# davidtweedle/gptq-svd

Hardware: AMD Instinct MI355X
Metric: weight-cols quantized/sec at d_in=4096 (higher is better)
Workload: dtype f64+f32; 1 GPU; single synthetic 4096x4096 Hessian per rank, full solver (eigh, rank rule, pivot order, U, 4-bit asym g128 quantize, pack); n=4096, m=4096, calib_rows=3072, rank_k=3058, threshold_method=energy, block_size=1024, parallelism=independent layer per rank x1

## Files before the change

### gptq-svd_amd/csrc/band.h

```cpp
#pragma once
#include <algorithm>
#include <type_traits>
#include <vector>

#include "common.h"

namespace tg {

constexpr int SB_B = 32;
constexpr int SB_C = 256;
constexpr int SB_LV = 6;
constexpr int PQR_NWMAX = 256;
constexpr int PQR_BC_DOUBLES = 8192;

struct SbLevel {
  int rows, nc;
  size_t yoff, toff;
};
struct SbPanel {
  int p, r0, m, nl;
  SbLevel L[SB_LV];
};

struct SbPlan {
  std::vector<SbPanel> panels;
  size_t ytotal = 0, ttotal = 0;
  int ncmax = 1;
  bool single = false;
  explicit SbPlan(int n);
};

struct SbBufs {
  double *Y, *T;
  double *YT, *X, *G, *M;
  double *YTl[SB_LV];
  double *R[2];
  double *Gr, *U;
  double *Xs;
  double *Zg, *P, *Mz;
  double *Bst;
  double *V2;
  double *T2;
  unsigned *prog;
  double *pq_part, *pq_bc;
  unsigned *pq_ctl;
  unsigned *xm_tick;
  double *xm_xpart;
};

int pqr_rows_per_thread(int m);
hipError_t panel_qr(hipStream_t st, double *A, int lda, int p, int r0, int m, double *Y,
                    double *YT, double *T, double *part, double *bc, unsigned *cnt,
                    unsigned *tmo);

int sb_smax(int n);
size_t sb2st_prog_words(int n);
size_t sb2st_t2_count(int n);

inline size_t pq_ctl_words(int n) { return 4 + 4 * size_t(std::max(1, n / SB_B + 1)); }
inline size_t xm_mflag_off(int n) { return size_t(n) / 256 + 7; }
inline size_t xm_cbt_off(int n) { return size_t(n) / 256 + 8; }
inline size_t xm_tick_words(int n) { return xm_cbt_off(n) + size_t(n) / 16 + 2; }
inline size_t xm_xpart_doubles(int n) { return 8 * (size_t(n) + 32) * 32; }

template <class A>
void sb_layout(A &ar, int n, int kmax, const SbPlan &pl, SbBufs *bp) {
  SbBufs d{};
  SbBufs &b = bp ? *bp : d;
  const size_t w = size_t(pl.ncmax) * SB_B;
  auto take = [&](double *&dst, size_t cnt) {
    if constexpr (std::is_same_v<A, Arena>) dst = ar.template take<double>(cnt);
    else ar.template take<double>(cnt);
  };
  take(b.Y, pl.ytotal + 1);
  take(b.T, pl.ttotal + 1);
  take(b.YT, size_t(n) * SB_B);
  for (int l = 1; l < SB_LV; ++l) take(b.YTl[l], w * SB_B);
  take(b.X, size_t(n) * w);
  take(b.G, w * w);
  take(b.M, w * w);
  take(b.R[0], w * SB_B);
  take(b.R[1], w * SB_B);
  take(b.Gr, w * n);
  take(b.U, std::max({w * n, (size_t(n) / 16 + size_t(n) / 256 + 2) * 1024,
                      (size_t(n) / 32 + size_t(n) / 1024 + 2) * 5 * 1024}));
  take(b.Xs, w * w);
  take(b.Zg, w * kmax);
  take(b.P, w * kmax);
  take(b.Mz, w * kmax);
  const size_t nsw = size_t(std::max(1, n - 2)), smax = size_t(sb_smax(n));
  take(b.Bst, size_t(n) * 2 * SB_B);
  take(b.V2, nsw * smax * SB_B);
  take(b.T2, sb2st_t2_count(n));
  if constexpr (std::is_same_v<A, Arena>) b.prog = ar.template take<unsigned>(sb2st_prog_words(n));
  else ar.template take<unsigned>(sb2st_prog_words(n));
  const size_t npart = std::max<size_t>(std::max<size_t>(2 * PQR_NWMAX + 2, size_t(n) / SB_C + 2),
                                        size_t(n) / 128 + 2) * 1024;
  take(b.pq_part, npart);
  take(b.pq_bc, PQR_BC_DOUBLES);
  if constexpr (std::is_same_v<A, Arena>) b.pq_ctl = ar.template take<unsigned>(pq_ctl_words(n));
  else ar.template take<unsigned>(pq_ctl_words(n));
  if constexpr (std::is_same_v<A, Arena>) b.xm_tick = ar.template take<unsigned>(xm_tick_words(n));
  else ar.template take<unsigned>(xm_tick_words(n));
  take(b.xm_xpart, xm_xpart_doubles(n));
}

hipError_t sy2sb(hipStream_t st, double *A, int lda, int n, const SbPlan &pl, const SbBufs &b);
hipError_t sy2sb_timed_out(hipStream_t st, const SbPlan &pl, const SbBufs &b, bool *tmo);
hipError_t sb2st(hipStream_t st, const double *A, int lda, int n, double *Bst, double *V2,
                 unsigned *prog, double *d, double *e);
hipError_t sb2st_stalled(hipStream_t st, int n, const unsigned *prog, bool *stalled,
                         bool *broken = nullptr);
hipError_t sb_apply_q2(hipStream_t st, int n, double *Z, int k, const double *V2,
                       double *T2);
hipError_t sb_q2_tfactors(hipStream_t st, int n, const double *V2, double *T2);
hipError_t side_fork(hipStream_t st, hipStream_t *side);
hipError_t side_join(hipStream_t st);
bool sb_apply_few_ok(const SbPlan &pl, int n, int k);
size_t sb_apply_few_scratch(const SbPlan &pl, int n, int k);
hipError_t sb_apply_few(hipStream_t st, int n, double *Z, int k, const SbPlan &pl,
                        const SbBufs &b, void *dev, bool *timed_out);
hipError_t sb_apply_q1(hipStream_t st, int n, double *Z, int k, const SbPlan &pl,
                       const SbBufs &b);

}
```

### gptq-svd_amd/csrc/band.hip

```cpp
#include <algorithm>
#include <cmath>
#include <cstdio>
#include <cstdlib>
#include <utility>
#include <vector>

#include "band.h"
#include "gemm64.h"
#include "reduce.h"
#include "spin.h"

namespace tg {

SbPlan::SbPlan(int n) {
  ncmax = std::max(1, n / SB_C);
  const char *e = getenv("TG_SB_TSQR");
  single = !(e && e[0] == '1') && pqr_rows_per_thread(n) > 0;
  int p = 0;
  while (p + SB_B < n - 1) {
    SbPanel P{};
    P.p = p;
    P.r0 = p + SB_B;
    P.m = n - P.r0;
    if (single) {
// ... 972 lines not shown
      if constexpr (NBC == 1)
        if (g.fuse_w) xm_fused_w<NBC>(g, r0, xs, ys, &red[XW - 4][0][0]);
      return;
    }
    for (int e = tid; e < ne; e += 64 * XW) Cs[e] = xm_sum(g.gpart, 0, NG, e, NP * 1024);
  }
  __syncthreads();
  for (int e = tid; e < SB_B * SB_B; e += 64 * XW) {
    const int a = e >> 5, c = e & 31;
    double v = 0.0;
    for (int k = 0; k <= a; ++k) v = fma(Ts[k * SB_B + a], Cs[k * SB_B + c], v);
    if (NBC == 1 && g.fuse_w)
      __hip_atomic_store(&g.M[e], v, __ATOMIC_RELAXED, __HIP_MEMORY_SCOPE_AGENT);
    else
      g.M[e] = v;
  }
  if (NBC == 1 && g.fuse_w) {
    asm volatile("s_waitcnt vmcnt(0)" ::: "memory");
    __syncthreads();
    if (tid == 0) {
      tg::ctl_reset(&g.tick[grp]);
      if (NG > 1) tg::ctl_reset(&g.tick[NG]);
      __hip_atomic_store(g.mflag, g.epoch, __ATOMIC_RELAXED, __HIP_MEMORY_SCOPE_AGENT);
    }
    if constexpr (NBC == 1) xm_fused_w<NBC>(g, r0, xs, ys, &red[XW - 4][0][0]);
    return;
  }
  if (pp) {
    const double *Ps = Cs + 1024, *Qs = Cs + 2048, *E1 = Cs + 3072, *E2 = Cs + 4096;
    for (int e = tid; e < 2048; e += 64 * XW) g.PQ[e] = Cs[1024 + e];
    __syncthreads();
    for (int e = tid; e < SB_B * SB_B; e += 64 * XW) {
      const int a = e >> 5, c = e & 31;
      double v = 0.0;
#pragma unroll 8
      for (int k = 0; k < SB_B; ++k) v = fma(E1[a * SB_B + k], Ps[k * SB_B + c], v);
#pragma unroll 8
      for (int k = 0; k < SB_B; ++k) v = fma(E2[a * SB_B + k], Qs[k * SB_B + c], v);
      Cs[e] = v;
    }
    __syncthreads();
    for (int e = tid; e < SB_B * SB_B; e += 64 * XW) {
      const int a = e >> 5, c = e & 31;
      double v = 0.0;
      for (int k = 0; k <= a; ++k) v = fma(Ts[k * SB_B + a], Cs[k * SB_B + c], v);
      g.PQ[2048 + e] = v;
    }
  }
  if (tid == 0) {
    tg::ctl_reset(&g.tick[grp]);
    if (NG > 1) tg::ctl_reset(&g.tick[NG]);
  }
}

constexpr int WU_R = 16;
__global__ __launch_bounds__(256) void w_update_kernel(const double *__restrict__ Y,
                                                       double *__restrict__ X, int m,
                                                       const double *__restrict__ M) {
  __shared__ double2 Ms[SB_B][SB_B / 2];
  const int tid = threadIdx.x;
  const int r = blockIdx.x * WU_R + (tid >> 4), c2 = tid & 15;
  const int rc = min(r, m - 1);
  double2 y[SB_B / 2];
#pragma unroll
  for (int h = 0; h < SB_B / 2; ++h) y[h] = reinterpret_cast<const double2 *>(Y + int64_t(rc) * SB_B)[h];
  const double2 x = reinterpret_cast<const double2 *>(X + int64_t(rc) * SB_B)[c2];
  for (int e = tid; e < SB_B * SB_B / 2; e += 256)
    Ms[e >> 4][e & 15] = reinterpret_cast<const double2 *>(M)[e];
  __syncthreads();
  double v0 = 0.0, v1 = 0.0;
#pragma unroll
  for (int h = 0; h < SB_B / 2; ++h) {
    const double2 a = Ms[2 * h][c2], b = Ms[2 * h + 1][c2];
    v0 = fma(y[h].x, a.x, v0);
    v1 = fma(y[h].x, a.y, v1);
    v0 = fma(y[h].y, b.x, v0);
    v1 = fma(y[h].y, b.y, v1);
  }
  if (r < m)
    reinterpret_cast<double2 *>(X + int64_t(r) * SB_B)[c2] =
        make_double2(fma(-0.5, v0, x.x), fma(-0.5, v1, x.y));
}

constexpr int WT = 64, WK = 2 * SB_B, WP = 4;
struct YW2 {
  const double *Y[2], *W[2];
};
template <int NP>
__global__ __launch_bounds__(256, 2) void syr2k_w_kernel(double *__restrict__ A, int64_t lda, int m,
                                                         YW2 yw) {
  __shared__ double Aop[WK][WT + WP];
  __shared__ double Bop[WK][WT + WP];
  const int b = blockIdx.x;
  int I = int((sqrt(8.0 * b + 1.0) - 1.0) * 0.5);
  while ((I + 1) * (I + 2) / 2 <= b) ++I;
  while (I * (I + 1) / 2 > b) --I;
  const int J = b - I * (I + 1) / 2;
  const int tm = I * WT, tn = J * WT;
  const int tid = threadIdx.x, lane = tid & 63, wid = tid >> 6;
  const int wm = wid >> 1, wn = wid & 1;
  double old[2][2][4];
#pragma unroll
  for (int i = 0; i < 2; ++i)
#pragma unroll
    for (int j = 0; j < 2; ++j)
#pragma unroll
      for (int r = 0; r < 4; ++r) {
        const int gi = min(tm + wm * 32 + i * 16 + (lane >> 4) + 4 * r, m - 1);
        const int gj = min(tn + wn * 32 + j * 16 + (lane & 15), m - 1);
        old[i][j][r] = A[int64_t(gi) * lda + gj];
      }
  doublex4 acc[2][2];
#pragma unroll
  for (int i = 0; i < 2; ++i)
#pragma unroll
    for (int j = 0; j < 2; ++j) acc[i][j] = doublex4{0.0, 0.0, 0.0, 0.0};
#pragma unroll
  for (int pp = 0; pp < NP; ++pp) {
    if (pp > 0) __syncthreads();
    const double *Y = yw.Y[pp], *W = yw.W[pp];
    {
      const int rl = tid >> 2, k0 = (tid & 3) * 8;
      const int gr = min(tm + rl, m - 1), gc = min(tn + rl, m - 1);
      const bool okr = tm + rl < m, okc = tn + rl < m;
      double2 v[4][4];
      const double *src[4] = {Y + int64_t(gr) * SB_B + k0, W + int64_t(gr) * SB_B + k0,
                              W + int64_t(gc) * SB_B + k0, Y + int64_t(gc) * SB_B + k0};
#pragma unroll
      for (int o = 0; o < 4; ++o)
#pragma unroll
        for (int h = 0; h < 4; ++h) v[o][h] = reinterpret_cast<const double2 *>(src[o])[h];
#pragma unroll
      for (int h = 0; h < 4; ++h) {
        const int k = k0 + 2 * h;
        Aop[k][rl] = okr ? v[0][h].x : 0.0;
        Aop[k + 1][rl] = okr ? v[0][h].y : 0.0;
        Aop[SB_B + k][rl] = okr ? v[1][h].x : 0.0;
        Aop[SB_B + k + 1][rl] = okr ? v[1][h].y : 0.0;
        Bop[k][rl] = okc ? v[2][h].x : 0.0;
        Bop[k + 1][rl] = okc ? v[2][h].y : 0.0;
        Bop[SB_B + k][rl] = okc ? v[3][h].x : 0.0;
        Bop[SB_B + k + 1][rl] = okc ? v[3][h].y : 0.0;
      }
    }
    __syncthreads();
#pragma unroll
    for (int kq = 0; kq < WK; kq += 4) {
      double af[2], bf[2];
#pragma unroll
      for (int i = 0; i < 2; ++i) af[i] = Aop[kq + (lane >> 4)][wm * 32 + i * 16 + (lane & 15)];
#pragma unroll
      for (int j = 0; j < 2; ++j) bf[j] = Bop[kq + (lane >> 4)][wn * 32 + j * 16 + (lane & 15)];
#pragma unroll
      for (int i = 0; i < 2; ++i)
#pragma unroll
        for (int j = 0; j < 2; ++j)
          acc[i][j] = __builtin_amdgcn_mfma_f64_16x16x4f64(af[i], bf[j], acc[i][j], 0, 0, 0);
    }
  }
  __syncthreads();
  double(*Tt)[WT + 1] = reinterpret_cast<double(*)[WT + 1]>(&Aop[0][0]);
  static_assert(WK * (WT + WP) >= WT * (WT + 1), "mirror tile must fit");
#pragma unroll
  for (int i = 0; i < 2; ++i)
#pragma unroll
    for (int j = 0; j < 2; ++j)
#pragma unroll
      for (int r = 0; r < 4; ++r) {
        const int li = wm * 32 + i * 16 + (lane >> 4) + 4 * r, lj = wn * 32 + j * 16 + (lane & 15);
        const int gi = tm + li, gj = tn + lj;
        if (gi < m && gj < m && gi >= gj) {
          const double v = old[i][j][r] - acc[i][j][r];
          A[int64_t(gi) * lda + gj] = v;
          if (tm != tn) Tt[li][lj] = v;
          else if (gi != gj) A[int64_t(gj) * lda + gi] = v;
        }
      }
  if (tm != tn) {
    __syncthreads();
    for (int idx = tid; idx < WT * WT; idx += 256) {
      const int lc = idx >> 6, lr = idx & 63;
      if (tn + lc < m && tm + lr < m) A[int64_t(tn + lc) * lda + tm + lr] = Tt[lr][lc];
    }
  }
}

__device__ __forceinline__ void syr2k_tile(int b, int &tm, int &tn) {
  int I = int((sqrt(8.0 * b + 1.0) - 1.0) * 0.5);
  while ((I + 1) * (I + 2) / 2 <= b) ++I;
  while (I * (I + 1) / 2 > b) --I;
  tm = I * WT;
  tn = (b - I * (I + 1) / 2) * WT;
}
template <int NP>
__global__ __launch_bounds__(256, 2) void syr2k_wp_kernel(double *__restrict__ A, int64_t lda,
                                                          int m, YW2 yw, int ntiles) {
  __shared__ double Aop[WK][WT + WP];
  __shared__ double Bop[WK][WT + WP];
  const int tid = threadIdx.x, lane = tid & 63, wid = tid >> 6;
  const int wm = wid >> 1, wn = wid & 1;
  int b = blockIdx.x;
  if (b >= ntiles) return;
  auto load_old = [&](int tb, double (&o)[2][2][4]) __attribute__((always_inline)) {
    int tm, tn;
    syr2k_tile(tb, tm, tn);
#pragma unroll
    for (int i = 0; i < 2; ++i)
#pragma unroll
      for (int j = 0; j < 2; ++j)
#pragma unroll
        for (int r = 0; r < 4; ++r) {
          const int gi = min(tm + wm * 32 + i * 16 + (lane >> 4) + 4 * r, m - 1);
          const int gj = min(tn + wn * 32 + j * 16 + (lane & 15), m - 1);
          o[i][j][r] = A[int64_t(gi) * lda + gj];
        }
  };
  double old[2][2][4], nold[2][2][4];
  load_old(b, old);
  for (; b < ntiles; b += gridDim.x) {
    int tm, tn;
    syr2k_tile(b, tm, tn);
    const int rl = tid >> 2, k0 = (tid & 3) * 8;
    const int gr = min(tm + rl, m - 1), gc = min(tn + rl, m - 1);
    const bool okr = tm + rl < m, okc = tn + rl < m;
    doublex4 acc[2][2];
#pragma unroll
    for (int i = 0; i < 2; ++i)
#pragma unroll
      for (int j = 0; j < 2; ++j) acc[i][j] = doublex4{0.0, 0.0, 0.0, 0.0};
#pragma unroll
    for (int pp = 0; pp < NP; ++pp) {
      __syncthreads();
      const double *Y = yw.Y[pp], *W = yw.W[pp];
      double2 v[4][4];
      {
        const double *src[4] = {Y + int64_t(gr) * SB_B + k0, W + int64_t(gr) * SB_B + k0,
                                W + int64_t(gc) * SB_B + k0, Y + int64_t(gc) * SB_B + k0};
#pragma unroll
        for (int o = 0; o < 4; ++o)
#pragma unroll
          for (int h = 0; h < 4; ++h) v[o][h] = reinterpret_cast<const double2 *>(src[o])[h];
      }
      if (pp == 0) {
        __builtin_amdgcn_sched_barrier(0);
        const int bn = b + int(gridDim.x);
        if (bn < ntiles) load_old(bn, nold);
        __builtin_amdgcn_sched_barrier(0);
      }
#pragma unroll
      for (int h = 0; h < 4; ++h) {
        const int k = k0 + 2 * h;
        Aop[k][rl] = okr ? v[0][h].x : 0.0;
        Aop[k + 1][rl] = okr ? v[0][h].y : 0.0;
        Aop[SB_B + k][rl] = okr ? v[1][h].x : 0.0;
        Aop[SB_B + k + 1][rl] = okr ? v[1][h].y : 0.0;
        Bop[k][rl] = okc ? v[2][h].x : 0.0;
        Bop[k + 1][rl] = okc ? v[2][h].y : 0.0;
        Bop[SB_B + k][rl] = okc ? v[3][h].x : 0.0;
        Bop[SB_B + k + 1][rl] = okc ? v[3][h].y : 0.0;
      }
      __syncthreads();
#pragma unroll
      for (int kq = 0; kq < WK; kq += 4) {
        double af[2], bf[2];
#pragma unroll
        for (int i = 0; i < 2; ++i) af[i] = Aop[kq + (lane >> 4)][wm * 32 + i * 16 + (lane & 15)];
#pragma unroll
        for (int j = 0; j < 2; ++j) bf[j] = Bop[kq + (lane >> 4)][wn * 32 + j * 16 + (lane & 15)];
#pragma unroll
        for (int i = 0; i < 2; ++i)
#pragma unroll
          for (int j = 0; j < 2; ++j)
            acc[i][j] = __builtin_amdgcn_mfma_f64_16x16x4f64(af[i], bf[j], acc[i][j], 0, 0, 0);
      }
    }
    __syncthreads();
// ... 266 lines not shown
  if (e != hipSuccess) return e;
  SideStream &x = ss[dev & 63];
  if (!x.s) {
    if ((e = hipStreamCreateWithFlags(&x.s, hipStreamNonBlocking)) != hipSuccess) return e;
    for (int i = 0; i < 2; ++i) {
      if ((e = hipEventCreateWithFlags(&x.ev0[i], hipEventDisableTiming)) != hipSuccess) return e;
      if ((e = hipEventCreateWithFlags(&x.ev1[i], hipEventDisableTiming)) != hipSuccess) return e;
    }
    if ((e = hipEventCreateWithFlags(&x.evj, hipEventDisableTiming)) != hipSuccess) return e;
  }
  out = &x;
  return hipSuccess;
}

hipError_t side_fork(hipStream_t st, hipStream_t *side) {
  SideStream *ss = nullptr;
  TG_CHK(side_stream(ss));
  TG_CHK(hipEventRecord(ss->evj, st));
  TG_CHK(hipStreamWaitEvent(ss->s, ss->evj, 0));
  *side = ss->s;
  return hipSuccess;
}
hipError_t side_join(hipStream_t st) {
  SideStream *ss = nullptr;
  TG_CHK(side_stream(ss));
  TG_CHK(hipEventRecord(ss->evj, ss->s));
  TG_CHK(hipStreamWaitEvent(st, ss->evj, 0));
  return hipSuccess;
}

static int xm_nbc(int m) {
  const char *fx = getenv("TG_XM_NBC");
  return fx ? (atoi(fx) == 2 ? 2 : 1) : (m >= XM_WIDE ? 2 : 1);
}
template <int NBC>
static int xm_resident() {
  static int cached[64] = {0};
  int dev = 0;
  if (hipGetDevice(&dev) != hipSuccess || dev < 0 || dev >= 64) return 0;
  if (cached[dev] == 0) {
    int ncu = 0, occ = 0;
    if (hipDeviceGetAttribute(&ncu, hipDeviceAttributeMultiprocessorCount, dev) != hipSuccess)
      ncu = 0;
    if (hipOccupancyMaxActiveBlocksPerMultiprocessor(&occ, xm_kernel<NBC>, 64 * XW, 0) !=
        hipSuccess)
      occ = 0;
    cached[dev] = std::max(0, ncu) * std::max(0, occ);
    if (cached[dev] == 0) cached[dev] = -1;
  }
  return std::max(0, cached[dev]);
}
static int xm_ksplit(int m, int G, int nbc) {
  const char *e = getenv("TG_XM_KSPLIT");
  int S = (e && atoi(e) > 0) ? atoi(e) : (nbc == 1 || G >= 1536 ? 1 : cdiv(1536, G));
  S = std::max(1, std::min(8, S));
  while (S > 1 && cdiv(m, S) < 4 * 32) --S;
  return S;
}
static hipError_t launch_xm(hipStream_t st, double *A22, int lda, int m, const double *YT,
                            const double *Yp, const double *Tp, double *X, const SbBufs &b,
                            int n, const double *Ya = nullptr, const double *Wa = nullptr,
                            double *PQ = nullptr, unsigned epoch = 0, bool *fused = nullptr) {
  const int nbc = xm_nbc(m);
  if (Ya && nbc != 2) return hipErrorInvalidValue;
  const int G = cdiv(m, XR * nbc), np = Ya ? 5 : 1;
  const int S = xm_ksplit(m, G, nbc), kc = cdiv(cdiv(m, S), 32) * 32;
  unsigned *mflag = b.xm_tick + xm_mflag_off(n);
  const char *xs = getenv("TG_XM_ASM");
  const int asm_loads = !(xs && xs[0] == '0');
  const char *fw = getenv("TG_XM_FUSE_W");
  const bool fuse = epoch > 0 && !Ya && nbc == 1 && (fw && fw[0] == '1') &&
                    2 * G * S <= xm_resident<1>();
  if (fused) *fused = fuse;
  static const unsigned long long tmo_ticks = spin_timeout_ticks("TG_XM_TIMEOUT_TICKS");
  XmArgs xa{A22, int64_t(lda), m, YT, Yp, Tp, X, b.U, b.U + size_t(G) * np * 1024, b.M,
            b.xm_tick, asm_loads, Ya, Wa, PQ, fuse ? 1 : 0,
            mflag, epoch, b.pq_ctl, tmo_ticks, S, kc, b.xm_xpart, b.xm_tick + xm_cbt_off(n)};
  if (nbc == 2) hipLaunchKernelGGL(xm_kernel<2>, dim3(G * S), dim3(64 * XW), 0, st, xa);
  else hipLaunchKernelGGL(xm_kernel<1>, dim3(G * S), dim3(64 * XW), 0, st, xa);
  return hipGetLastError();
}

constexpr int PAIR_MIN_ALL = 256, PAIR_MIN = 6144;

static hipError_t sy2sb_single(hipStream_t st, double *A, int lda, int n, const SbPlan &pl,
                               const SbBufs &b) {
  TG_CHK(hipMemsetAsync(b.pq_ctl, 0, sizeof(unsigned) * pq_ctl_words(n), st));
  TG_CHK(hipMemsetAsync(b.xm_tick, 0, sizeof(unsigned) * xm_tick_words(n), st));
  const int np = int(pl.panels.size());
  const char *pe = getenv("TG_SB_PAIR");
  const bool pairs = !(pe && pe[0] == '0') && pl.ncmax >= 2;
  const int pair_min = (pe && pe[0] == '1') ? PAIR_MIN_ALL : PAIR_MIN;
  const char *ps = getenv("TG_SYR2K_PERSIST");
  const bool persist = !(ps && ps[0] == '0');
  const XcdInfo xi = xcd_info();
  const int ncu = std::max(1, xi.xcds * xi.cus_per_xcd);
  SideStream *ss = nullptr;
  const char *psd = getenv("TG_SB_PAIR_SIDE");
  const bool pair_side = psd && psd[0] == '1';
  double *Xa = b.X, *Xb = b.X + size_t(n) * SB_B;
  for (int pi = 0; pi < np; ++pi) {
    const SbPanel &P = pl.panels[pi];
    const int m = P.m, r0 = P.r0;
    double *A22 = A + int64_t(r0) * lda + r0;
    double *Yp = b.Y + P.L[0].yoff, *Tp = b.T + P.L[0].toff;
    TG_CHK(panel_qr(st, A, lda, P.p, P.r0, P.m, Yp, b.YT, Tp, b.pq_part, b.pq_bc,
                    b.pq_ctl + 4 + 4 * pi, b.pq_ctl));
    const bool pair = pairs && pi + 1 < np && pl.panels[pi + 1].m >= pair_min;
    bool fused = false;
    TG_CHK(launch_xm(st, A22, lda, m, b.YT, Yp, Tp, Xa, b, n, nullptr, nullptr, nullptr,
                     unsigned(pi + 1), &fused));
    if (!fused) {
      hipLaunchKernelGGL(w_update_kernel, dim3(cdiv(m, WU_R)), dim3(256), 0, st, Yp, Xa, m, b.M);
      TG_CHK(hipGetLastError());
    }
    if (!pair) {
      const int nt = cdiv(m, WT), tiles = nt * (nt + 1) / 2;
      auto tok = prof_begin(st, PROF_SBUPD, 12.0 * double(m) * m, 64.0 * double(m) * m);
      if (persist)
        hipLaunchKernelGGL(syr2k_wp_kernel<1>, dim3(std::min(tiles, 2 * ncu)), dim3(256), 0, st,
                           A22, int64_t(lda), m, YW2{{Yp, nullptr}, {Xa, nullptr}}, tiles);
      else
        hipLaunchKernelGGL(syr2k_w_kernel<1>, dim3(tiles), dim3(256), 0, st, A22, int64_t(lda), m,
                           YW2{{Yp, nullptr}, {Xa, nullptr}});
      prof_end(st, tok);
      TG_CHK(hipGetLastError());
      continue;
    }
    hipLaunchKernelGGL(panel_upd_kernel, dim3(cdiv(m, SB_B)), dim3(256), 0, st, A22,
                       int64_t(lda), m, Yp, Xa);
    TG_CHK(hipGetLastError());
    ++pi;
    const SbPanel &Q = pl.panels[pi];
    const int mb = Q.m;
    double *A22b = A + int64_t(Q.r0) * lda + Q.r0;
    double *Yb = b.Y + Q.L[0].yoff, *Tb = b.T + Q.L[0].toff;
    const double *Ya = Yp + SB_B * SB_B, *Wa = Xa + SB_B * SB_B;
    TG_CHK(panel_qr(st, A, lda, Q.p, Q.r0, Q.m, Yb, b.YT, Tb, b.pq_part, b.pq_bc,
                    b.pq_ctl + 4 + 4 * pi, b.pq_ctl));
    if (xm_nbc(mb) == 2 && !pair_side) {
      TG_CHK(launch_xm(st, A22b, lda, mb, b.YT, Yb, Tb, Xb, b, n, Ya, Wa, b.G));
    } else {
      const int nblk = cdiv(mb, PR);
      if (!ss) TG_CHK(side_stream(ss));
      TG_CHK(hipEventRecord(ss->ev0[0], st));
      TG_CHK(hipStreamWaitEvent(ss->s, ss->ev0[0], 0));
      hipLaunchKernelGGL(pair_part_kernel, dim3(nblk), dim3(256), 0, ss->s, Ya, Wa, Yb, b.YT, mb,
                         b.Gr);
      TG_CHK(hipGetLastError());
      hipLaunchKernelGGL(pair_fin_kernel, dim3(1), dim3(1024), 0, ss->s, b.Gr, nblk, Tb, b.G);
      TG_CHK(hipGetLastError());
      TG_CHK(hipEventRecord(ss->ev1[0], ss->s));
      TG_CHK(launch_xm(st, A22b, lda, mb, b.YT, Yb, Tb, Xb, b, n));
      TG_CHK(hipStreamWaitEvent(st, ss->ev1[0], 0));
    }
    hipLaunchKernelGGL(w_update2_kernel, dim3(cdiv(mb, WU_R)), dim3(256), 0, st, Yb, Xb, mb, b.M,
                       Ya, Wa, b.G);
    TG_CHK(hipGetLastError());
    const int nt = cdiv(mb, WT);
    auto tok = prof_begin(st, PROF_SBUPD, 12.0 * double(mb) * mb, 128.0 * double(mb) * mb);
    const int tiles = nt * (nt + 1) / 2;
    if (persist)
      hipLaunchKernelGGL(syr2k_wp_kernel<2>, dim3(std::min(tiles, 2 * ncu)), dim3(256), 0, st,
                         A22b, int64_t(lda), mb, YW2{{Ya, Yb}, {Wa, Xb}}, tiles);
    else
      hipLaunchKernelGGL(syr2k_w_kernel<2>, dim3(tiles), dim3(256), 0, st, A22b, int64_t(lda), mb,
                         YW2{{Ya, Yb}, {Wa, Xb}});
    prof_end(st, tok);
    TG_CHK(hipGetLastError());
  }
  return hipSuccess;
}

hipError_t sy2sb_timed_out(hipStream_t st, const SbPlan &pl, const SbBufs &b, bool *tmo) {
  *tmo = false;
  if (!pl.single || pl.panels.empty()) return hipSuccess;
  unsigned h = 0;
  hipError_t e = hipMemcpyAsync(&h, b.pq_ctl, sizeof(unsigned), hipMemcpyDeviceToHost, st);
  if (e == hipSuccess) e = hipStreamSynchronize(st);
  *tmo = h != 0u;
  if (getenv("TG_PQR_STATS")) {
    std::vector<unsigned> c(4 + 4 * pl.panels.size());
    (void)hipMemcpy(c.data(), b.pq_ctl, sizeof(unsigned) * c.size(), hipMemcpyDeviceToHost);
    int hist[4][NPQ_STAT] = {};
    for (size_t i = 0; i < pl.panels.size(); ++i) {
      const unsigned v = c[4 + 4 * i + 1];
      hist[std::min(3u, v / 16)][std::min(unsigned(NPQ_STAT - 1), v % 16)]++;
    }
    fprintf(stderr, "pqr: %zu panels; accept after 2/3/4 passes: %d/%d/%d; fallback: %d\n",
            pl.panels.size(), hist[2][2], hist[2][3], hist[2][4],
            hist[3][0] + hist[3][1] + hist[3][2] + hist[3][3] + hist[3][4]);
  }
  return e;
}

hipError_t sy2sb(hipStream_t st, double *A, int lda, int n, const SbPlan &pl, const SbBufs &b) {
  if (pl.single) return sy2sb_single(st, A, lda, n, pl, b);
  SideStream *ss = nullptr;
  TG_CHK(side_stream(ss));
  int pi = 0;
  for (const SbPanel &P : pl.panels) {
    const int m = P.m, r0 = P.r0;
    double *A22 = A + int64_t(r0) * lda + r0;
    RowMap mp{};
    for (int l = 0; l < P.nl; ++l) mp.nc[l] = P.L[l].nc;
    TG_CHK(launch_qr(st, A + int64_t(r0) * lda + P.p, lda, P.L[0].nc, m, b.Y + P.L[0].yoff,
                     b.T + P.L[0].toff, b.R[0], b.YT));
    const int ph = pi & 1;
// ... 122 lines not shown
```

### gptq-svd_amd/csrc/pqr.hip

```cpp
#include <algorithm>
#include <cfloat>
#include <cmath>
#include <cstdio>
#include <cstdlib>
#include <utility>

#include "band.h"
#include "common.h"
#include "spin.h"
#include "lanes.h"

namespace {

using tg::SB_B;
constexpr int PT = 256;
constexpr int XS = 34;
constexpr int NPASS = 4;
constexpr int FB_MIN_M = 64;
constexpr double SERIES_TOL = 1e-5;

enum Dec { DEC_CONTINUE = 1, DEC_ACCEPT = 2, DEC_FALLBACK = 3 };

constexpr int BC_DEC = 0, BC_L = 64, BC_RINV = BC_L + 1024, BC_T = BC_RINV + 64,
              BC_PROW = BC_T + 1024, BC_MB = BC_PROW + 128, BC_SIZE = BC_MB + 2048;
// ... 730 lines not shown
                                                    : (npass >= NPASS ? DEC_FALLBACK : DEC_CONTINUE);
    if (lane == 0) sm.dec = d;
  }
  __syncthreads();
  DBG_STAMP(dk + 2)
  const int d = sm.dec;
  if (d != DEC_FALLBACK) {
    if (npass == 1) {
      for (int e = tid; e < 1024; e += PT) sm.Ra[e >> 5][e & 31] = sm.Lt[e >> 5][e & 31];
    } else {
      mm32<33, 33, 33>(&sm.RgI[0][0], &sm.Lt[0][0], &sm.Ra[0][0], nullptr);
      __syncthreads();
      for (int e = tid; e < 1024; e += PT) sm.Ra[e >> 5][e & 31] = sm.RgI[e >> 5][e & 31];
    }
    __syncthreads();
  }
  DBG_STAMP(dk + 3)
  if (d == DEC_ACCEPT) {
    DBG_STAMP(dk + 4)
    hr_top_ool();
    DBG_STAMP(dk + 5)
    for (int e = tid; e < 2048; e += PT) st_sc1(g.bc + BC_MB + e, sm.MB[e >> 6][e & 63]);
    for (int e = tid; e < 1024; e += PT) g.T[e] = sm.Tm[e >> 5][e & 31];
  }
  if (d == DEC_CONTINUE) {
    for (int e = tid; e < 1024; e += PT) st_sc1(g.bc + BC_L + e, sm.Lt[e >> 5][e & 31]);
    if (tid < 32) st_sc1(g.bc + BC_RINV + tid, sm.rinv[tid]);
  }
  DBG_STAMP(dk + 6)
  if (tid == 0) {
    st_sc1(g.bc + BC_DEC, double(d));
    tg::ctl_record(g.cnt + 1, unsigned(d * 16 + npass));
  }
  return d;
}

__device__ __forceinline__ void ph_apply(int w) {
  PqrSm &sm = s_pq;
  const PqrArgs &g = sm.ga;
  const int tid = otid();
  if (w != 0) {
    double t[4];
#pragma unroll
    for (int u = 0; u < 4; ++u) t[u] = ld_sc1(g.bc + BC_L + tid + PT * u);
    const double ri = tid < 32 ? ld_sc1(g.bc + BC_RINV + tid) : 0.0;
#pragma unroll
    for (int u = 0; u < 4; ++u) {
      const int e = tid + PT * u;
      sm.Lt[e >> 5][e & 31] = t[u];
    }
    if (tid < 32) sm.rinv[tid] = ri;
    __syncthreads();
  }
  double x[32];
  row_from_lds(&sm.Xs[tid][0], x);
  trsm_row(x, sm.Lt, sm.rinv);
  row_to_lds(&sm.Xs[tid][0], x);
  __syncthreads();
}

__device__ __forceinline__ void ph_final(int w) {
  PqrSm &sm = s_pq;
  const PqrArgs &g = sm.ga;
  const int tid = otid();
  if (w != 0) {
    double t[8];
#pragma unroll
    for (int u = 0; u < 8; ++u) t[u] = ld_sc1(g.bc + BC_MB + tid + PT * u);
#pragma unroll
    for (int u = 0; u < 8; ++u) {
      const int e = tid + PT * u;
      sm.MB[e >> 6][e & 63] = t[u];
    }
    __syncthreads();
  }
  final_rows(g, sm, w);
}

__device__ __noinline__ void ph_householder(int w, unsigned ep) {
  unsigned e = ep;
  householder(s_pq.ga, s_pq, w, e);
}

__global__ __launch_bounds__(PT) void pqr_kernel(PqrArgs ga) {
  PqrSm &sm = s_pq;
  if (blockIdx.x % ga.wstride != 0) return;
  const int w = blockIdx.x / ga.wstride;
  const int tid = otid();
  if (tid == 0) sm.ga = ga;
  unsigned ep = 0;
  int nst = 0;
  auto stamp = [&]() {
    if (ga.stats && w == 0 && tid == 0 && nst < 15) ga.stats[nst] = __builtin_amdgcn_s_memrealtime();
    ++nst;
  };
  stamp();
  int dec = (ga.m < FB_MIN_M || ga.force_fb) ? DEC_FALLBACK : DEC_CONTINUE;
  if (dec == DEC_CONTINUE) {
    double x[32];
    load_row(ga, w * PT + tid, x);
    row_to_lds(&sm.Xs[tid][0], x);
  }
  __syncthreads();
  int npass = 0;
  while (dec == DEC_CONTINUE) {
    ph_gram(w);
    stamp();
    ph_bar(++ep);
    stamp();
    ++npass;
    if (w == 0) ph_decide(npass);
    stamp();
    ph_bar(++ep);
    stamp();
    dec = int(ld_sc1(ga.bc + BC_DEC));
    if (dec == DEC_ACCEPT) {
      ph_final(w);
      stamp();
      return;
    }
    if (dec == DEC_CONTINUE) ph_apply(w);
  }
  ph_householder(w, ep);
}

}

namespace tg {

static int pqr_resident_workers() {
  static int cached[64] = {0};
  int dev = 0;
  if (hipGetDevice(&dev) != hipSuccess || dev < 0 || dev >= 64) return 0;
  if (cached[dev] == 0) {
    int ncu = 0, occ = 0;
    if (hipDeviceGetAttribute(&ncu, hipDeviceAttributeMultiprocessorCount, dev) != hipSuccess)
      ncu = 0;
    if (hipOccupancyMaxActiveBlocksPerMultiprocessor(&occ, pqr_kernel, PT, 0) != hipSuccess)
      occ = 0;
    cached[dev] = std::max(0, ncu) * std::max(0, occ);
    if (cached[dev] == 0) cached[dev] = -1;
  }
  return std::max(0, cached[dev]);
}

int pqr_rows_per_thread(int m) {
  return m <= PQR_NWMAX * PT && cdiv(m, PT) <= pqr_resident_workers() ? 1 : 0;
}

hipError_t panel_qr(hipStream_t st, double *A, int lda, int p, int r0, int m, double *Y,
                    double *YT, double *T, double *part, double *bc, unsigned *cnt,
                    unsigned *tmo) {
  if (m < 1 || pqr_rows_per_thread(m) == 0) return hipErrorInvalidValue;
  PqrArgs g{};
  g.A = A;
  g.lda = lda;
  g.p = p;
  g.r0 = r0;
  g.m = m;
  g.nw = cdiv(m, PT);
  g.Y = Y;
  g.YT = YT;
  g.T = T;
  g.part = part;
  g.bc = bc;
  g.cnt = cnt;
  g.tmo = tmo;
  static const unsigned long long tmo_ticks = spin_timeout_ticks("TG_PQR_TIMEOUT_TICKS");
  g.timeout = tmo_ticks;
  {
    const char *fb = getenv("TG_PQR_FALLBACK");
    g.force_fb = (fb && fb[0] == '1') ? 1 : 0;
  }
  static unsigned long long *stats = nullptr;
  static int nstat = 0;
  static double acc[16] = {0};
  if (getenv("TG_PQR_STATS")) {
    if (!stats) {
      (void)hipMalloc(&stats, 16 * sizeof(unsigned long long));
      atexit([] {
        if (nstat == 0) return;
        fprintf(stderr, "pqr phases (us, mean of %d accepted 2-pass panels):", nstat);
        for (int i = 1; i < 10; ++i) fprintf(stderr, " %.2f", acc[i] / nstat / 100.0);
        fprintf(stderr, "\n");
      });
    }
    (void)hipMemsetAsync(stats, 0, 16 * sizeof(unsigned long long), st);
    g.stats = stats;
  }
  auto tok = prof_begin(st, PROF_TSQR, 8.0 * m * SB_B * 3, 10.0 * m * SB_B * SB_B);
  const XcdInfo xi = xcd_info();
  g.wstride = g.nw <= xi.cus_per_xcd ? xi.xcds : 1;
  hipLaunchKernelGGL(pqr_kernel, dim3(g.wstride * g.nw), dim3(PT), 0, st, g);
  prof_end(st, tok);
  if (g.stats) {
    unsigned long long h[16];
    (void)hipMemcpyAsync(h, g.stats, sizeof(h), hipMemcpyDeviceToHost, st);
    (void)hipStreamSynchronize(st);
    if (h[9] != 0 && h[10] == 0) {
      for (int i = 1; i < 10; ++i) acc[i] += double(h[i] - h[i - 1]);
      ++nstat;
    }
#ifdef TG_PQR_DBG
    static int ndbg = 0;
    if (++ndbg == 250) {
      unsigned long long d[64];
      (void)hipMemcpyFromSymbol(d, HIP_SYMBOL(g_pq_dbg), sizeof(d));
      fprintf(stderr, "pqr decide sub-phases (us, sums over launches): p1 reduce %.1f chol %.1f ra %.1f pub %.1f | p2 reduce %.1f chol %.1f ra %.1f cq %.1f hr %.1f pub %.1f\n",
              (d[1] - d[0]) / 100.0, (d[2] - d[1]) / 100.0, (d[3] - d[2]) / 100.0, (d[6] - d[3]) / 100.0,
              (d[9] - d[8]) / 100.0, (d[10] - d[9]) / 100.0, (d[11] - d[10]) / 100.0,
              (d[12] - d[11]) / 100.0, (d[13] - d[12]) / 100.0, (d[14] - d[13]) / 100.0);
      fprintf(stderr, "  shifted first passes: %llu; chol32: loop %.1f tail %.1f (sums)\n", d[30],
              (d[25] - d[24]) / 100.0, (d[26] - d[25]) / 100.0);
      fprintf(stderr, "  hr: LU||RgI %.1f  T||UI||R %.1f  M1+Y1T %.1f  (sums); LU %.1f RgI %.1f\n",
              (d[17] - d[16]) / 100.0, (d[18] - d[17]) / 100.0, (d[19] - d[18]) / 100.0,
              (d[20] - d[16]) / 100.0, (d[21] - d[16]) / 100.0);
    }
#endif
  }
  return hipGetLastError();
}

}
```

Before: 68850 cols/s.

## Fuse trailing syr2k update with next panel QR in one persistent kernel

Adds a persistent kernel that performs the SYR2K trailing-matrix update and then, on designated blocks, runs the next panel's QR once the first tile-column has been written. The first column of tiles is stored write-through and counted, so QR workers can spin on that counter while other blocks finish the rest of the update. This removes a kernel launch boundary per panel and lets panel QR overlap the remaining update work. It applies only for large panels (m >= 5120) unless overridden by environment. In exchange it adds spin-wait synchronisation, shared-memory overlays and a dynamic tile-ticket scheduler, which can deadlock or time out if fewer blocks are resident than the code assumes.

```diff
diff --git a/gptq-svd_amd/csrc/band.h b/gptq-svd_amd/csrc/band.h
--- a/gptq-svd_amd/csrc/band.h
+++ b/gptq-svd_amd/csrc/band.h
@@ -52,6 +52,24 @@
 hipError_t panel_qr(hipStream_t st, double *A, int lda, int p, int r0, int m, double *Y,
                     double *YT, double *T, double *part, double *bc, unsigned *cnt,
                     unsigned *tmo);
+struct PanelQr {
+  double *A;
+  int lda, p, r0, m;
+  double *Y, *YT, *T, *part, *bc;
+  unsigned *cnt, *tmo;
+};
+
+constexpr int SYR2K_WT = 64, SYR2K_WP = 4;
+__device__ __forceinline__ void syr2k_tile(int b, int &tm, int &tn) {
+  int I = int((sqrt(8.0 * b + 1.0) - 1.0) * 0.5);
+  while ((I + 1) * (I + 2) / 2 <= b) ++I;
+  while (I * (I + 1) / 2 > b) --I;
+  tm = I * SYR2K_WT;
+  tn = (b - I * (I + 1) / 2) * SYR2K_WT;
+}
+int syr2k_panel_qr_grid(int m);
+hipError_t syr2k_panel_qr(hipStream_t st, double *A22, int lda, int m, const double *Y,
+                          const double *W, const PanelQr &q);
 
 int sb_smax(int n);
 size_t sb2st_prog_words(int n);
diff --git a/gptq-svd_amd/csrc/band.hip b/gptq-svd_amd/csrc/band.hip
--- a/gptq-svd_amd/csrc/band.hip
+++ b/gptq-svd_amd/csrc/band.hip
@@ -1078,7 +1078,8 @@
         make_double2(fma(-0.5, v0, x.x), fma(-0.5, v1, x.y));
 }
 
-constexpr int WT = 64, WK = 2 * SB_B, WP = 4;
+constexpr int WT = tg::SYR2K_WT, WK = 2 * SB_B, WP = tg::SYR2K_WP;
+using tg::syr2k_tile;
 struct YW2 {
   const double *Y[2], *W[2];
 };
@@ -1181,13 +1182,6 @@
   }
 }
 
-__device__ __forceinline__ void syr2k_tile(int b, int &tm, int &tn) {
-  int I = int((sqrt(8.0 * b + 1.0) - 1.0) * 0.5);
-  while ((I + 1) * (I + 2) / 2 <= b) ++I;
-  while (I * (I + 1) / 2 > b) --I;
-  tm = I * WT;
-  tn = (b - I * (I + 1) / 2) * WT;
-}
 template <int NP>
 __global__ __launch_bounds__(256, 2) void syr2k_wp_kernel(double *__restrict__ A, int64_t lda,
                                                           int m, YW2 yw, int ntiles) {
@@ -1620,6 +1614,7 @@
 }
 
 constexpr int PAIR_MIN_ALL = 256, PAIR_MIN = 6144;
+constexpr int FUSE_QR_MIN_M = 5120;
 
 static hipError_t sy2sb_single(hipStream_t st, double *A, int lda, int n, const SbPlan &pl,
                                const SbBufs &b) {
@@ -1637,13 +1632,19 @@
   const char *psd = getenv("TG_SB_PAIR_SIDE");
   const bool pair_side = psd && psd[0] == '1';
   double *Xa = b.X, *Xb = b.X + size_t(n) * SB_B;
+  const char *fq = getenv("TG_SB_FUSE_QR");
+  const bool fuse_all = fq && fq[0] == '1';
+  const bool fuse_any = persist && !(fq && fq[0] == '0');
+  bool qr_done = false;
   for (int pi = 0; pi < np; ++pi) {
     const SbPanel &P = pl.panels[pi];
     const int m = P.m, r0 = P.r0;
     double *A22 = A + int64_t(r0) * lda + r0;
     double *Yp = b.Y + P.L[0].yoff, *Tp = b.T + P.L[0].toff;
-    TG_CHK(panel_qr(st, A, lda, P.p, P.r0, P.m, Yp, b.YT, Tp, b.pq_part, b.pq_bc,
-                    b.pq_ctl + 4 + 4 * pi, b.pq_ctl));
+    if (!qr_done)
+      TG_CHK(panel_qr(st, A, lda, P.p, P.r0, P.m, Yp, b.YT, Tp, b.pq_part, b.pq_bc,
+                      b.pq_ctl + 4 + 4 * pi, b.pq_ctl));
+    qr_done = false;
     const bool pair = pairs && pi + 1 < np && pl.panels[pi + 1].m >= pair_min;
     bool fused = false;
     TG_CHK(launch_xm(st, A22, lda, m, b.YT, Yp, Tp, Xa, b, n, nullptr, nullptr, nullptr,
@@ -1655,13 +1656,23 @@
     if (!pair) {
       const int nt = cdiv(m, WT), tiles = nt * (nt + 1) / 2;
       auto tok = prof_begin(st, PROF_SBUPD, 12.0 * double(m) * m, 64.0 * double(m) * m);
-      if (persist)
+      hipError_t fe = hipSuccess;
+      if (fuse_any && pi + 1 < np && (fuse_all || m >= FUSE_QR_MIN_M) &&
+          syr2k_panel_qr_grid(m) > 0) {
+        const SbPanel &Q = pl.panels[pi + 1];
+        fe = syr2k_panel_qr(st, A22, lda, m, Yp, Xa,
+                            PanelQr{A, lda, Q.p, Q.r0, Q.m, b.Y + Q.L[0].yoff, b.YT,
+                                    b.T + Q.L[0].toff, b.pq_part, b.pq_bc,
+                                    b.pq_ctl + 4 + 4 * (pi + 1), b.pq_ctl});
+        qr_done = true;
+      } else if (persist)
         hipLaunchKernelGGL(syr2k_wp_kernel<1>, dim3(std::min(tiles, 2 * ncu)), dim3(256), 0, st,
                            A22, int64_t(lda), m, YW2{{Yp, nullptr}, {Xa, nullptr}}, tiles);
       else
         hipLaunchKernelGGL(syr2k_w_kernel<1>, dim3(tiles), dim3(256), 0, st, A22, int64_t(lda), m,
                            YW2{{Yp, nullptr}, {Xa, nullptr}});
       prof_end(st, tok);
+      TG_CHK(fe);
       TG_CHK(hipGetLastError());
       continue;
     }
diff --git a/gptq-svd_amd/csrc/pqr.hip b/gptq-svd_amd/csrc/pqr.hip
--- a/gptq-svd_amd/csrc/pqr.hip
+++ b/gptq-svd_amd/csrc/pqr.hip
@@ -836,10 +836,8 @@
   householder(s_pq.ga, s_pq, w, e);
 }
 
-__global__ __launch_bounds__(PT) void pqr_kernel(PqrArgs ga) {
+__device__ __forceinline__ void pqr_body(const PqrArgs &ga, int w) {
   PqrSm &sm = s_pq;
-  if (blockIdx.x % ga.wstride != 0) return;
-  const int w = blockIdx.x / ga.wstride;
   const int tid = otid();
   if (tid == 0) sm.ga = ga;
   unsigned ep = 0;
@@ -878,6 +876,213 @@
   ph_householder(w, ep);
 }
 
+__global__ __launch_bounds__(PT) void pqr_kernel(PqrArgs ga) {
+  if (blockIdx.x % ga.wstride != 0) return;
+  pqr_body(ga, blockIdx.x / ga.wstride);
+}
+
+constexpr int WT = tg::SYR2K_WT, WK = 2 * SB_B, WP = tg::SYR2K_WP;
+static_assert(sizeof(PqrSm::Xs) >= 2 * WK * (WT + WP) * sizeof(double), "operand images overlay Xs");
+static_assert(WK * (WT + WP) >= WT * (WT + 1), "mirror tile must fit");
+
+struct FuseArgs {
+  double *A22;
+  int64_t lda;
+  int m, nt, ntiles;
+  const double *Y, *W;
+  PqrArgs q;
+  unsigned long long *fstats;
+};
+
+__shared__ int s_ticket;
+
+template <bool THROUGH>
+__device__ __forceinline__ void tile_put(double *p, double v) {
+  if constexpr (THROUGH) st_sc1(p, v);
+  else *p = v;
+}
+
+template <bool THROUGH>
+__device__ __forceinline__ void tile_store(double *A, int64_t lda, int m, int tm, int tn,
+                                           const double (&old)[2][2][4],
+                                           const doublex4 (&acc)[2][2], double (*Tt)[WT + 1]) {
+  const int tid = threadIdx.x, lane = tid & 63, wid = tid >> 6, wm = wid >> 1, wn = wid & 1;
+#pragma unroll
+  for (int i = 0; i < 2; ++i)
+#pragma unroll
+    for (int j = 0; j < 2; ++j)
+#pragma unroll
+      for (int r = 0; r < 4; ++r) {
+        const int li = wm * 32 + i * 16 + (lane >> 4) + 4 * r, lj = wn * 32 + j * 16 + (lane & 15);
+        const int gi = tm + li, gj = tn + lj;
+        if (gi < m && gj < m && gi >= gj) {
+          const double val = old[i][j][r] - acc[i][j][r];
+          tile_put<THROUGH>(A + int64_t(gi) * lda + gj, val);
+          if (tm != tn) Tt[li][lj] = val;
+          else if (gi != gj) tile_put<THROUGH>(A + int64_t(gj) * lda + gi, val);
+        }
+      }
+  if (tm != tn) {
+    __syncthreads();
+    for (int idx = tid; idx < WT * WT; idx += PT) {
+      const int lc = idx >> 6, lr = idx & 63;
+      if (tn + lc < m && tm + lr < m)
+        tile_put<THROUGH>(A + int64_t(tn + lc) * lda + tm + lr, Tt[lr][lc]);
+    }
+  }
+}
+
+__global__ __launch_bounds__(PT) void syr2k_pqr_kernel(FuseArgs fa) {
+  PqrSm &sm = s_pq;
+  double(*Aop)[WT + WP] = reinterpret_cast<double(*)[WT + WP]>(&sm.Xs[0][0]);
+  double(*Bop)[WT + WP] = Aop + WK;
+  double(*Tt)[WT + 1] = reinterpret_cast<double(*)[WT + 1]>(&sm.Xs[0][0]);
+  double *A = fa.A22;
+  const int64_t lda = fa.lda;
+  const int m = fa.m, nt = fa.nt, ntiles = fa.ntiles, G = int(gridDim.x);
+  const int tid = threadIdx.x, lane = tid & 63, wid = tid >> 6;
+  const int wm = wid >> 1, wn = wid & 1;
+  const bool wave0 = __builtin_amdgcn_readfirstlane(wid) == 0;
+  unsigned *tick = fa.q.cnt + 2, *done = fa.q.cnt + 3;
+  const int qw = int(blockIdx.x) / fa.q.wstride;
+  bool qr_due = int(blockIdx.x) % fa.q.wstride == 0 && qw < fa.q.nw;
+  auto tile_of = [&](int t, int &tm, int &tn) __attribute__((always_inline)) {
+    if (t < nt) {
+      tm = t * WT;
+      tn = 0;
+    } else {
+      tg::syr2k_tile(t - nt, tm, tn);
+      tm += WT;
+      tn += WT;
+    }
+  };
+  auto load_old = [&](int t, double (&o)[2][2][4]) __attribute__((always_inline)) {
+    int tm, tn;
+    tile_of(t, tm, tn);
+#pragma unroll
+    for (int i = 0; i < 2; ++i)
+#pragma unroll
+      for (int j = 0; j < 2; ++j)
+#pragma unroll
+        for (int r = 0; r < 4; ++r) {
+          const int gi = min(tm + wm * 32 + i * 16 + (lane >> 4) + 4 * r, m - 1);
+          const int gj = min(tn + wn * 32 + j * 16 + (lane & 15), m - 1);
+          o[i][j][r] = A[int64_t(gi) * lda + gj];
+        }
+  };
+  auto fstamp = [&](int k) {
+    if (fa.fstats && blockIdx.x == 0 && tid == 0) fa.fstats[k] = __builtin_amdgcn_s_memrealtime();
+  };
+  fstamp(0);
+  double old[2][2][4], nold[2][2][4];
+  int cur = int(blockIdx.x);
+  bool have_old = false;
+  for (;;) {
+    if (cur < ntiles) {
+      if (!have_old) load_old(cur, old);
+      const bool look = !qr_due;
+      int tm, tn;
+      tile_of(cur, tm, tn);
+      const int rl = tid >> 2, k0 = (tid & 3) * 8;
+      const int gr = min(tm + rl, m - 1), gc = min(tn + rl, m - 1);
+      const bool okr = tm + rl < m, okc = tn + rl < m;
+      doublex4 acc[2][2];
+#pragma unroll
+      for (int i = 0; i < 2; ++i)
+#pragma unroll
+        for (int j = 0; j < 2; ++j) acc[i][j] = doublex4{0.0, 0.0, 0.0, 0.0};
+      __syncthreads();
+      unsigned tk = 0;
+      if (look && tid == 0)
+        tk = __hip_atomic_fetch_add((gu32 *)tick, 1u, __ATOMIC_RELAXED, __HIP_MEMORY_SCOPE_AGENT);
+      double2 v[4][4];
+      {
+        const double *src[4] = {fa.Y + int64_t(gr) * SB_B + k0, fa.W + int64_t(gr) * SB_B + k0,
+                                fa.W + int64_t(gc) * SB_B + k0, fa.Y + int64_t(gc) * SB_B + k0};
+#pragma unroll
+        for (int o = 0; o < 4; ++o)
+#pragma unroll
+          for (int h = 0; h < 4; ++h) v[o][h] = reinterpret_cast<const double2 *>(src[o])[h];
+      }
+#pragma unroll
+      for (int h = 0; h < 4; ++h) {
+        const int k = k0 + 2 * h;
+        Aop[k][rl] = okr ? v[0][h].x : 0.0;
+        Aop[k + 1][rl] = okr ? v[0][h].y : 0.0;
+        Aop[SB_B + k][rl] = okr ? v[1][h].x : 0.0;
+        Aop[SB_B + k + 1][rl] = okr ? v[1][h].y : 0.0;
+        Bop[k][rl] = okc ? v[2][h].x : 0.0;
+        Bop[k + 1][rl] = okc ? v[2][h].y : 0.0;
+        Bop[SB_B + k][rl] = okc ? v[3][h].x : 0.0;
+        Bop[SB_B + k + 1][rl] = okc ? v[3][h].y : 0.0;
+      }
+      if (look && tid == 0) s_ticket = G + int(tk);
+      __syncthreads();
+      int nxt = ntiles;
+      if (look) {
+        nxt = __builtin_amdgcn_readfirstlane(s_ticket);
+        __builtin_amdgcn_sched_barrier(0);
+        if (nxt < ntiles) load_old(nxt, nold);
+        __builtin_amdgcn_sched_barrier(0);
+      }
+#pragma unroll
+      for (int kq = 0; kq < WK; kq += 4) {
+        double af[2], bf[2];
+#pragma unroll
+        for (int i = 0; i < 2; ++i) af[i] = Aop[kq + (lane >> 4)][wm * 32 + i * 16 + (lane & 15)];
+#pragma unroll
+        for (int j = 0; j < 2; ++j) bf[j] = Bop[kq + (lane >> 4)][wn * 32 + j * 16 + (lane & 15)];
+#pragma unroll
+        for (int i = 0; i < 2; ++i)
+#pragma unroll
+          for (int j = 0; j < 2; ++j)
+            acc[i][j] = __builtin_amdgcn_mfma_f64_16x16x4f64(af[i], bf[j], acc[i][j], 0, 0, 0);
+      }
+      __syncthreads();
+      if (tn == 0) {
+        tile_store<true>(A, lda, m, tm, tn, old, acc, Tt);
+        asm volatile("s_waitcnt vmcnt(0)" ::: "memory");
+        __syncthreads();
+        if (wave0) tg::wave_arrive(done);
+      } else {
+        tile_store<false>(A, lda, m, tm, tn, old, acc, Tt);
+      }
+      if (look) {
+        cur = nxt;
+        have_old = nxt < ntiles;
+#pragma unroll
+        for (int i = 0; i < 2; ++i)
+#pragma unroll
+          for (int j = 0; j < 2; ++j)
+#pragma unroll
+            for (int r = 0; r < 4; ++r) old[i][j][r] = nold[i][j][r];
+        continue;
+      }
+    } else if (!qr_due) {
+      break;
+    }
+    fstamp(1);
+    if (wave0) {
+      tg::spin_geq(done, unsigned(nt), fa.q.tmo, fa.q.timeout);
+      __builtin_amdgcn_fence(__ATOMIC_ACQUIRE, "agent");
+      asm volatile("s_waitcnt vmcnt(0)" ::: "memory");
+    }
+    __syncthreads();
+    fstamp(2);
+    pqr_body(fa.q, qw);
+    qr_due = false;
+    __syncthreads();
+    fstamp(3);
+    if (tid == 0)
+      s_ticket = G + int(__hip_atomic_fetch_add((gu32 *)tick, 1u, __ATOMIC_RELAXED,
+                                                __HIP_MEMORY_SCOPE_AGENT));
+    __syncthreads();
+    cur = __builtin_amdgcn_readfirstlane(s_ticket);
+    have_old = false;
+  }
+  fstamp(4);
+}
+
 }
 
 namespace tg {
@@ -902,30 +1107,108 @@
   return m <= PQR_NWMAX * PT && cdiv(m, PT) <= pqr_resident_workers() ? 1 : 0;
 }
 
+static PqrArgs pqr_args(const PanelQr &q) {
+  PqrArgs g{};
+  g.A = q.A;
+  g.lda = q.lda;
+  g.p = q.p;
+  g.r0 = q.r0;
+  g.m = q.m;
+  g.nw = cdiv(q.m, PT);
+  g.Y = q.Y;
+  g.YT = q.YT;
+  g.T = q.T;
+  g.part = q.part;
+  g.bc = q.bc;
+  g.cnt = q.cnt;
+  g.tmo = q.tmo;
+  static const unsigned long long tmo_ticks = spin_timeout_ticks("TG_PQR_TIMEOUT_TICKS");
+  g.timeout = tmo_ticks;
+  const char *fb = getenv("TG_PQR_FALLBACK");
+  g.force_fb = (fb && fb[0] == '1') ? 1 : 0;
+  const XcdInfo xi = xcd_info();
+  g.wstride = g.nw <= xi.cus_per_xcd ? xi.xcds : 1;
+  return g;
+}
+
+static int fuse_resident() {
+  static int cached[64] = {0};
+  int dev = 0;
+  if (hipGetDevice(&dev) != hipSuccess || dev < 0 || dev >= 64) return 0;
+  if (cached[dev] == 0) {
+    int ncu = 0, occ = 0;
+    if (hipDeviceGetAttribute(&ncu, hipDeviceAttributeMultiprocessorCount, dev) != hipSuccess)
+      ncu = 0;
+    if (hipOccupancyMaxActiveBlocksPerMultiprocessor(&occ, syr2k_pqr_kernel, PT, 0) != hipSuccess)
+      occ = 0;
+    cached[dev] = std::max(0, ncu) * std::max(0, occ);
+    if (cached[dev] == 0) cached[dev] = -1;
+  }
+  return std::max(0, cached[dev]);
+}
+
+int syr2k_panel_qr_grid(int m) {
+  const int mq = m - SB_B;
+  if (mq < 1 || pqr_rows_per_thread(mq) == 0) return 0;
+  const XcdInfo xi = xcd_info();
+  const int nw = cdiv(mq, PT), ws = nw <= xi.cus_per_xcd ? xi.xcds : 1;
+  const int nt = cdiv(m, WT), cap = fuse_resident();
+  const long long tiles = (long long)nt * (nt + 1) / 2;
+  const int G = std::max(int(std::min<long long>(tiles, cap)), ws * (nw - 1) + 1);
+  return (G <= cap && nt <= G) ? G : 0;
+}
+
+hipError_t syr2k_panel_qr(hipStream_t st, double *A22, int lda, int m, const double *Y,
+                          const double *W, const PanelQr &q) {
+  const int G = syr2k_panel_qr_grid(m);
+  if (G == 0 || q.m != m - SB_B || q.lda != lda) return hipErrorInvalidValue;
+  FuseArgs fa{};
+  fa.A22 = A22;
+  fa.lda = lda;
+  fa.m = m;
+  fa.nt = cdiv(m, WT);
+  fa.ntiles = fa.nt * (fa.nt + 1) / 2;
+  fa.Y = Y;
+  fa.W = W;
+  fa.q = pqr_args(q);
+  static unsigned long long *stats = nullptr;
+  static int nstat = 0;
+  static double acc[16] = {0}, facc[4] = {0};
+  if (getenv("TG_PQR_STATS")) {
+    if (!stats) {
+      (void)hipMalloc(&stats, 24 * sizeof(unsigned long long));
+      atexit([] {
+        if (nstat == 0) return;
+        fprintf(stderr, "fused update + pqr (us, mean of %d accepted 2-pass panels): first tile %.2f "
+                        "column 0 %.2f qr %.2f tail %.2f | pqr phases:", nstat, facc[0] / nstat / 100.0,
+                facc[1] / nstat / 100.0, facc[2] / nstat / 100.0, facc[3] / nstat / 100.0);
+        for (int i = 1; i < 10; ++i) fprintf(stderr, " %.2f", acc[i] / nstat / 100.0);
+        fprintf(stderr, "\n");
+      });
+    }
+    (void)hipMemsetAsync(stats, 0, 24 * sizeof(unsigned long long), st);
+    fa.q.stats = stats;
+    fa.fstats = stats + 16;
+  }
+  hipLaunchKernelGGL(syr2k_pqr_kernel, dim3(G), dim3(PT), 0, st, fa);
+  if (fa.fstats) {
+    unsigned long long h[24];
+    (void)hipMemcpyAsync(h, stats, sizeof(h), hipMemcpyDeviceToHost, st);
+    (void)hipStreamSynchronize(st);
+    if (h[9] != 0 && h[10] == 0) {
+      for (int i = 1; i < 10; ++i) acc[i] += double(h[i] - h[i - 1]);
+      for (int i = 0; i < 4; ++i) facc[i] += double(h[17 + i] - h[16 + i]);
+      ++nstat;
+    }
+  }
+  return hipGetLastError();
+}
+
 hipError_t panel_qr(hipStream_t st, double *A, int lda, int p, int r0, int m, double *Y,
                     double *YT, double *T, double *part, double *bc, unsigned *cnt,
                     unsigned *tmo) {
   if (m < 1 || pqr_rows_per_thread(m) == 0) return hipErrorInvalidValue;
-  PqrArgs g{};
-  g.A = A;
-  g.lda = lda;
-  g.p = p;
-  g.r0 = r0;
-  g.m = m;
-  g.nw = cdiv(m, PT);
-  g.Y = Y;
-  g.YT = YT;
-  g.T = T;
-  g.part = part;
-  g.bc = bc;
-  g.cnt = cnt;
-  g.tmo = tmo;
-  static const unsigned long long tmo_ticks = spin_timeout_ticks("TG_PQR_TIMEOUT_TICKS");
-  g.timeout = tmo_ticks;
-  {
-    const char *fb = getenv("TG_PQR_FALLBACK");
-    g.force_fb = (fb && fb[0] == '1') ? 1 : 0;
-  }
+  PqrArgs g = pqr_args(PanelQr{A, lda, p, r0, m, Y, YT, T, part, bc, cnt, tmo});
   static unsigned long long *stats = nullptr;
   static int nstat = 0;
   static double acc[16] = {0};
@@ -943,8 +1226,6 @@
     g.stats = stats;
   }
   auto tok = prof_begin(st, PROF_TSQR, 8.0 * m * SB_B * 3, 10.0 * m * SB_B * SB_B);
-  const XcdInfo xi = xcd_info();
-  g.wstride = g.nw <= xi.cus_per_xcd ? xi.xcds : 1;
   hipLaunchKernelGGL(pqr_kernel, dim3(g.wstride * g.nw), dim3(PT), 0, st, g);
   prof_end(st, tok);
   if (g.stats) {
```

New measurement: 68600 cols/s. About the same (-0.4%).
